# ViV99/slam-experiments

Measured on AMD Instinct MI355X. Metric: descriptor pairs/sec BF-Hamming knn=2 @64kx64k, higher is better.
Workload: dtype u32

## Files before the change

slam-experiments_amd/csrc/bf_mx32.hip:

```cpp
#include "internal.h"
#include <type_traits>

#include "bf_common.h"
#include "bf_mx_common.h"

typedef float mx_v16f __attribute__((ext_vector_type(16)));

__device__ __forceinline__ mx_v16f mx32_dot(uint4 a, uint4 b, mx_v16f c) {
    const mx_v8i av = {(int)a.x, (int)a.y, (int)a.z, (int)a.w, 0, 0, 0, 0};
    const mx_v8i bv = {(int)b.x, (int)b.y, (int)b.z, (int)b.w, 0, 0, 0, 0};
    return __builtin_amdgcn_mfma_scale_f32_32x32x64_f8f6f4(av, bv, c, 4, 4, 0, 0, 0, 0);
}

#define MX32_GROUP 32
#define MX32_GROUPS (SLAM_MX_STAGE / MX32_GROUP)

__global__ __launch_bounds__(256) __attribute__((amdgpu_waves_per_eu(4, 4))) void bf_top2_mx32_kernel(
    const uint4* __restrict__ q, int N, const uint4* __restrict__ t, const int* __restrict__ tbl, bf_state st, int train_base,
    int2* __restrict__ out_idx, int2* __restrict__ out_dist, uint4* __restrict__ keep, int nchunks, bf_select sel) {
    __shared__ uint4 tile[2][SLAM_MX_STAGE * 8];
    __shared__ u32 s_ticket, s_last;
    const int tid = threadIdx.x;
    const int lane = tid & 63, wave = tid >> 6;
    const int hk = lane >> 5, col = lane & 31;
    const int bx = ((int)blockIdx.x + (int)blockIdx.y) % (int)gridDim.x;
    auto lane_query = [&]() -> int {
        int v = tid;
        asm volatile("" : "+v"(v));
        return bx * 256 + v;
    };

    uint4 qb[2][4];
    const u32* qw = (const u32*)q;
#pragma unroll
    for (int tt = 0; tt < 2; tt++) {
        int qi = bx * 256 + wave * 64 + tt * 32 + col;
        qi = qi < N ? qi : N - 1;
#pragma unroll
        for (int kq = 0; kq < 4; kq++) qb[tt][kq] = mx_expand(qw[(size_t)qi * 8 + kq * 2 + hk]);
    }
    if (const int qbase = lane_query(); keep && blockIdx.y == 0 && qbase < N) {
        keep[2 * (size_t)qbase] = q[2 * (size_t)qbase];
        keep[2 * (size_t)qbase + 1] = q[2 * (size_t)qbase + 1];
    }

    u32 b1[2], b2[2], xs[2];
    int thr[2];
    auto set_threshold = [&](int tt, u32 x) {
        xs[tt] = x;
        thr[tt] = x > 129u ? (int)0x80000000u : __float_as_int((float)(258 - 2 * (int)x));
    };
#pragma unroll
    for (int tt = 0; tt < 2; tt++) {
        b1[tt] = b2[tt] = SLAM_KEY_NONE;
        set_threshold(tt, SLAM_KEY_NONE >> SLAM_KEY_IDX_BITS);
    }
    auto unite_tile = [&](int tt, u32& u1, u32& u2) {
        u1 = b1[tt];
        u2 = b2[tt];
        const u32 c1 = (u32)__shfl_xor((int)u1, 32, 64), c2 = (u32)__shfl_xor((int)u2, 32, 64);
        mx_unite(u1, u2, c1, c2);
    };
    u32 gkey = SLAM_BOUND_IDLE, pend[1] = {0u};
    auto exchange = [&](int c0) {
        u32 u1[2], u2[2];
#pragma unroll
        for (int tt = 0; tt < 2; tt++) unite_tile(tt, u1[tt], u2[tt]);
        if (const int qbase = lane_query(); qbase < N) {
            const u32 own = hk ? u2[1] : u2[0];
            asm volatile("" ::"v"(pend[0]));
            const u32 g = __hip_atomic_load(&st.bound[qbase], __ATOMIC_RELAXED, __HIP_MEMORY_SCOPE_AGENT);
            if (own < g && own < SLAM_MX_BOUND_LIMIT) pend[0] = atomicMin(&st.bound[qbase], own);
            gkey = g;
        }
#pragma unroll
        for (int tt = 0; tt < 2; tt++) {
            const u32 g = (u32)__shfl((int)gkey, tt * 32 + col, 64);
            set_threshold(tt, min(xs[tt], min(mx_bound_x(g, c0), u2[tt] >> SLAM_KEY_IDX_BITS)));
        }
    };

    const int srow = tid >> 1, sh = tid & 1;
    auto load_stage = [&](int s, int c1) -> uint4 {
        const uint4* ts = t + 2 * (size_t)s;
        if (s + SLAM_MX_STAGE <= c1) return ts[(u32)tid];
        return s + srow < c1 ? ts[(u32)tid] : make_uint4(0, 0, 0, 0);
    };
    const u32 fill = 0x22222222u;
    uint4* const dst0 = tile[0] + (srow >> 5) * 256 + sh * 128 + (srow & 31);
    auto store_word = [&](uint4* dst, int j, u32 v) { dst[(j >> 1) * 64 + (j & 1) * 32] = mx_expand_op(v, fill); };
    auto store_stage = [&](int b, uint4 v) {
        uint4* dst = dst0 + b * (SLAM_MX_STAGE * 8);
        store_word(dst, 0, v.x);
        store_word(dst, 1, v.y);
        store_word(dst, 2, v.z);
        store_word(dst, 3, v.w);
    };

    u32* const cursor = st.cursor + (size_t)(4 * bx) * SLAM_CURSOR_STRIDE;
    if (tid == 0) s_ticket = __hip_atomic_fetch_add(cursor, 1u, __ATOMIC_RELAXED, __HIP_MEMORY_SCOPE_AGENT);
    __syncthreads();
    int ci = __builtin_amdgcn_readfirstlane((int)s_ticket);
    int scanned = 0;
    while (ci < nchunks) {
        const int c0 = tbl[ci], c1 = tbl[ci + 1];
        const uint4 first = load_stage(c0, c1);
        exchange(c0);
        store_stage(0, first);
        __syncthreads();
        int buf = 0;
        for (int s0 = c0; s0 < c1; s0 += SLAM_MX_STAGE) {
            const int s1 = s0 + SLAM_MX_STAGE;
            const bool more = s1 < c1;
            if (!more && tid == 0) s_ticket = __hip_atomic_fetch_add(cursor, 1u, __ATOMIC_RELAXED, __HIP_MEMORY_SCOPE_AGENT);
            const uint4* tp = tile[buf];
            u32 fired = 0;
            auto fold = [&](int g, const mx_v16f (&acc)[2], auto rag) {
                int m[2];
#pragma unroll
                for (int tt = 0; tt < 2; tt++) {
                    int p = max(max(__float_as_int(acc[tt][0]), __float_as_int(acc[tt][1])), __float_as_int(acc[tt][2]));
#pragma unroll
                    for (int i = 3; i < 15; i += 2) p = max(max(p, __float_as_int(acc[tt][i])), __float_as_int(acc[tt][i + 1]));
                    m[tt] = max(p, __float_as_int(acc[tt][15]));
                }
                if (__builtin_expect(__ballot(m[0] >= thr[0] || m[1] >= thr[1]) != 0ull, 0)) {
                    int row0 = s0 + g * MX32_GROUP;
                    asm("" : "+s"(row0));
                    const u32 rowk = (u32)row0 + (u32)(4 * hk);
#pragma unroll
                    for (int tt = 0; tt < 2; tt++) {
                        if (__ballot(m[tt] >= thr[tt]) == 0ull) continue;
                        fired |= 1u << tt;
                        const u32 base = (128u << SLAM_KEY_IDX_BITS) + rowk;
#pragma unroll
                        for (int i = 0; i < 16; i++) {
                            if (__ballot(__float_as_int(acc[tt][i]) >= thr[tt]) == 0ull) continue;
                            const int off = 8 * (i >> 2) + (i & 3);
                            u32 key = base + (u32)off + ((u32)(int)(-acc[tt][i]) << (SLAM_KEY_IDX_BITS - 1));
                            if constexpr (decltype(rag)::value)
                                key = (int)rowk + off < c1 ? key : SLAM_KEY_NONE;
                            b2[tt] = umed3(b1[tt], b2[tt], key);
                            b1[tt] = min(b1[tt], key);
                        }
                        set_threshold(tt, min(xs[tt], b2[tt] >> SLAM_KEY_IDX_BITS));
                    }
                }
            };
            const mx_v16f zero = {0, 0, 0, 0, 0, 0, 0, 0, 0, 0, 0, 0, 0, 0, 0, 0};
            auto group = [&](int g, auto rag) {
                mx_v16f acc[2];
#pragma unroll
                for (int kq = 0; kq < 4; kq++) {
                    const uint4 a = tp[g * 256 + kq * 64 + lane];
#pragma unroll
                    for (int tt = 0; tt < 2; tt++) acc[tt] = mx32_dot(a, qb[tt][kq], kq ? acc[tt] : zero);
                }
                fold(g, acc, rag);
            };
            auto trip = [&](auto shadow) {
                constexpr bool SH = decltype(shadow)::value;
                const uint4* ap = tp + lane;
                uint4* const dst = dst0 + (buf ^ 1) * (SLAM_MX_STAGE * 8);
                u32 nx[4] = {0, 0, 0, 0};
                if (SH) {
                    const uint4 x = (t + 2 * (size_t)s1)[2 * min(srow, c1 - 1 - s1) + sh];
                    nx[0] = x.x; nx[1] = x.y; nx[2] = x.z; nx[3] = x.w;
                }
                uint4 a[4];
#pragma unroll
                for (int kq = 0; kq < 4; kq++) a[kq] = ap[kq * 64];
#pragma unroll
                for (int k = 0; k < MX32_GROUPS; k++) {
                    mx_v16f acc[2];
#pragma unroll
                    for (int kq = 0; kq < 4; kq++) {
                        __builtin_amdgcn_sched_barrier(0);
#pragma unroll
                        for (int tt = 0; tt < 2; tt++) acc[tt] = mx32_dot(a[kq], qb[tt][kq], kq ? acc[tt] : zero);
                        __builtin_amdgcn_sched_barrier(0);
                        if (k + 1 < MX32_GROUPS) a[kq] = ap[(k + 1) * 256 + kq * 64];
                        if (SH && k >= 1 && kq == 1) store_word(dst, k - 1, nx[k - 1]);
                        if (SH && k == 3 && kq == 2) store_word(dst, 3, nx[3]);
                    }
                    __builtin_amdgcn_sched_barrier(0);
                    fold(k, acc, std::false_type{});
                    __builtin_amdgcn_sched_barrier(0);
                }
            };
            if (more) {
                trip(std::true_type{});
            } else if (s1 == c1) {
                trip(std::false_type{});
            } else {
                const int ng = __builtin_amdgcn_readfirstlane((c1 - s0 + MX32_GROUP - 1) / MX32_GROUP);
                for (int g = 0; g < ng; g++) group(g, std::true_type{});
            }
#pragma unroll
            for (int tt = 0; tt < 2; tt++) {
                if (!(fired >> tt & 1u)) continue;
                u32 u1, u2;
                unite_tile(tt, u1, u2);
                set_threshold(tt, min(xs[tt], u2 >> SLAM_KEY_IDX_BITS));
            }
            scanned += min(s1, c1) - s0;
            if (more && scanned < 32 * SLAM_MX_STAGE && (SLAM_MX_EARLY >> (scanned / SLAM_MX_STAGE) & 1u)) exchange(s1);
            __syncthreads();
            buf ^= 1;
        }
        ci = __builtin_amdgcn_readfirstlane((int)s_ticket);
    }

    u32 u1[2], u2[2];
#pragma unroll
    for (int tt = 0; tt < 2; tt++) unite_tile(tt, u1[tt], u2[tt]);
    const u32 f1[1] = {hk ? u1[1] : u1[0]}, f2[1] = {hk ? u2[1] : u2[0]};
    const u32 gk[1] = {gkey < SLAM_MX_BOUND_LIMIT ? gkey >> SLAM_KEY_IDX_BITS : SLAM_BOUND_IDLE};
    bf_top2_epilogue<1, true>(st, bx, tid, lane, lane_query(), false, false, f1, f2, gk, pend, N, (int)gridDim.y, train_base, out_idx,
                              out_dist, sel, s_last);
}
```

Before: 11320 billion.

## Software-pipeline MFMA tiles so each tile's fold overlaps the other tile's dots

```diff
diff --git a/slam-experiments_amd/csrc/bf_mx32.hip b/slam-experiments_amd/csrc/bf_mx32.hip
--- a/slam-experiments_amd/csrc/bf_mx32.hip
+++ b/slam-experiments_amd/csrc/bf_mx32.hip
@@ -115,37 +115,34 @@
             if (!more && tid == 0) s_ticket = __hip_atomic_fetch_add(cursor, 1u, __ATOMIC_RELAXED, __HIP_MEMORY_SCOPE_AGENT);
             const uint4* tp = tile[buf];
             u32 fired = 0;
-            auto fold = [&](int g, const mx_v16f (&acc)[2], auto rag) {
-                int m[2];
-#pragma unroll
-                for (int tt = 0; tt < 2; tt++) {
-                    int p = max(max(__float_as_int(acc[tt][0]), __float_as_int(acc[tt][1])), __float_as_int(acc[tt][2]));
-#pragma unroll
-                    for (int i = 3; i < 15; i += 2) p = max(max(p, __float_as_int(acc[tt][i])), __float_as_int(acc[tt][i + 1]));
-                    m[tt] = max(p, __float_as_int(acc[tt][15]));
-                }
-                if (__builtin_expect(__ballot(m[0] >= thr[0] || m[1] >= thr[1]) != 0ull, 0)) {
-                    int row0 = s0 + g * MX32_GROUP;
-                    asm("" : "+s"(row0));
-                    const u32 rowk = (u32)row0 + (u32)(4 * hk);
-#pragma unroll
-                    for (int tt = 0; tt < 2; tt++) {
-                        if (__ballot(m[tt] >= thr[tt]) == 0ull) continue;
-                        fired |= 1u << tt;
-                        const u32 base = (128u << SLAM_KEY_IDX_BITS) + rowk;
-#pragma unroll
-                        for (int i = 0; i < 16; i++) {
-                            if (__ballot(__float_as_int(acc[tt][i]) >= thr[tt]) == 0ull) continue;
-                            const int off = 8 * (i >> 2) + (i & 3);
-                            u32 key = base + (u32)off + ((u32)(int)(-acc[tt][i]) << (SLAM_KEY_IDX_BITS - 1));
-                            if constexpr (decltype(rag)::value)
-                                key = (int)rowk + off < c1 ? key : SLAM_KEY_NONE;
-                            b2[tt] = umed3(b1[tt], b2[tt], key);
-                            b1[tt] = min(b1[tt], key);
-                        }
-                        set_threshold(tt, min(xs[tt], b2[tt] >> SLAM_KEY_IDX_BITS));
-                    }
-                }
+            auto fold_tile = [&](int tt, int g, const mx_v16f& acc, auto rag) {
+                int p = max(max(__float_as_int(acc[0]), __float_as_int(acc[1])), __float_as_int(acc[2]));
+#pragma unroll
+                for (int i = 3; i < 15; i += 2) p = max(max(p, __float_as_int(acc[i])), __float_as_int(acc[i + 1]));
+                const int m = max(p, __float_as_int(acc[15]));
+                if (__builtin_expect(__ballot(m >= thr[tt]) == 0ull, 1)) return;
+                fired |= 1u << tt;
+                int row0 = s0 + g * MX32_GROUP;
+                asm("" : "+s"(row0));
+                const u32 rowk = (u32)row0 + (u32)(4 * hk);
+                const u32 base = (128u << SLAM_KEY_IDX_BITS) + rowk;
+                unsigned long long gate[16];
+#pragma unroll
+                for (int i = 0; i < 16; i++) gate[i] = __ballot(__float_as_int(acc[i]) >= thr[tt]);
+                asm volatile("" ::"s"(gate[0]), "s"(gate[1]), "s"(gate[2]), "s"(gate[3]), "s"(gate[4]), "s"(gate[5]), "s"(gate[6]),
+                             "s"(gate[7]), "s"(gate[8]), "s"(gate[9]), "s"(gate[10]), "s"(gate[11]), "s"(gate[12]), "s"(gate[13]),
+                             "s"(gate[14]), "s"(gate[15]));
+#pragma unroll
+                for (int i = 0; i < 16; i++) {
+                    if (gate[i] == 0ull) continue;
+                    const int off = 8 * (i >> 2) + (i & 3);
+                    u32 key = base + (u32)off + ((u32)(int)(-acc[i]) << (SLAM_KEY_IDX_BITS - 1));
+                    if constexpr (decltype(rag)::value)
+                        key = (int)rowk + off < c1 ? key : SLAM_KEY_NONE;
+                    b2[tt] = umed3(b1[tt], b2[tt], key);
+                    b1[tt] = min(b1[tt], key);
+                }
+                set_threshold(tt, min(xs[tt], b2[tt] >> SLAM_KEY_IDX_BITS));
             };
             const mx_v16f zero = {0, 0, 0, 0, 0, 0, 0, 0, 0, 0, 0, 0, 0, 0, 0, 0};
             auto group = [&](int g, auto rag) {
@@ -156,7 +153,8 @@
 #pragma unroll
                     for (int tt = 0; tt < 2; tt++) acc[tt] = mx32_dot(a, qb[tt][kq], kq ? acc[tt] : zero);
                 }
-                fold(g, acc, rag);
+#pragma unroll
+                for (int tt = 0; tt < 2; tt++) fold_tile(tt, g, acc[tt], rag);
             };
             auto trip = [&](auto shadow) {
                 constexpr bool SH = decltype(shadow)::value;
@@ -170,23 +168,37 @@
                 uint4 a[4];
 #pragma unroll
                 for (int kq = 0; kq < 4; kq++) a[kq] = ap[kq * 64];
+                mx_v16f acc[2];
+                auto dot = [&](int tt, int kq) {
+                    __builtin_amdgcn_sched_barrier(0);
+                    acc[tt] = mx32_dot(a[kq], qb[tt][kq], kq ? acc[tt] : zero);
+                    __builtin_amdgcn_sched_barrier(0);
+                };
 #pragma unroll
                 for (int k = 0; k < MX32_GROUPS; k++) {
-                    mx_v16f acc[2];
-#pragma unroll
-                    for (int kq = 0; kq < 4; kq++) {
+                    auto ahead = [&](int kq) {
+                        if (k + 1 < MX32_GROUPS) a[kq] = ap[(k + 1) * 256 + kq * 64];
                         __builtin_amdgcn_sched_barrier(0);
-#pragma unroll
-                        for (int tt = 0; tt < 2; tt++) acc[tt] = mx32_dot(a[kq], qb[tt][kq], kq ? acc[tt] : zero);
-                        __builtin_amdgcn_sched_barrier(0);
-                        if (k + 1 < MX32_GROUPS) a[kq] = ap[(k + 1) * 256 + kq * 64];
-                        if (SH && k >= 1 && kq == 1) store_word(dst, k - 1, nx[k - 1]);
-                        if (SH && k == 3 && kq == 2) store_word(dst, 3, nx[3]);
-                    }
-                    __builtin_amdgcn_sched_barrier(0);
-                    fold(k, acc, std::false_type{});
-                    __builtin_amdgcn_sched_barrier(0);
-                }
+                    };
+                    dot(0, 0);
+                    dot(0, 1);
+                    dot(0, 2);
+                    dot(0, 3);
+                    if (k) fold_tile(1, k - 1, acc[1], std::false_type{});
+                    dot(1, 0);
+                    ahead(0);
+                    dot(1, 1);
+                    ahead(1);
+                    if (SH && k >= 1) store_word(dst, k - 1, nx[k - 1]);
+                    dot(1, 2);
+                    ahead(2);
+                    if (SH && k == 3) store_word(dst, 3, nx[3]);
+                    dot(1, 3);
+                    ahead(3);
+                    fold_tile(0, k, acc[0], std::false_type{});
+                }
+                __builtin_amdgcn_sched_barrier(0);
+                fold_tile(1, MX32_GROUPS - 1, acc[1], std::false_type{});
             };
             if (more) {
                 trip(std::true_type{});
```

Result: faster. 11720 billion, median of 6 (+3.5%).
